# roryhighnam/iib_project_ldpc_codes

Measured on AMD Instinct MI355X. Metric: decoded codewords/sec + info-bit Gb/s, (3,6) n=10k 50-iter BP, 1/2/4/8 MI355X, higher is better.
Workload: dtype f32

## Files before the change

iib_project_ldpc_codes_amd/csrc/bp_loc.hpp:

```cpp
#pragma once
#include "bp_device.hpp"

namespace ldpc {
namespace {

#ifndef LDPC_LOC_VGROUP
#define LDPC_LOC_VGROUP 1
#endif
#ifndef LDPC_LOC_CGROUP
#define LDPC_LOC_CGROUP 1
#endif
template <int N, int D>
__device__ __forceinline__ uint32_t bits_parity(const float2 (&x)[D], bool hi, uint32_t seed) {
    auto w = [&](int j) { return __float_as_uint(hi ? x[j].y : x[j].x); };
    uint32_t p = seed;
    int j = 2;
#pragma unroll
    for (; j + 1 < N; j += 2) p = xor3u(p, w(j), w(j + 1));
    if (j < N) p ^= w(j);
    return p;
}
template <int D, int ALGO, bool MIXED = false, bool SGN = false, int CL = 0>
__device__ __forceinline__ int loc_check_pair(float *msg, int W, int Nc, int i, float2 &l0, float2 &l1, float alpha,
                                              uint32_t lpar = 0u, float2 *chain = nullptr) {
    constexpr int C = CL > 0 ? 1 : 0, U = D - 2 - C;
    float2 x[D];
    x[0] = l0;
    x[1] = l1;
    if constexpr (C) x[2] = *chain;
#pragma unroll
    for (int r = 0; r < U / 2; ++r) {
        const float4 f = *reinterpret_cast<const float4 *>(msg + W + r * 4 * Nc + 4 * i);
        x[2 + C + 2 * r] = make_float2(f.x, f.y);
        x[3 + C + 2 * r] = make_float2(f.z, f.w);
    }
    if constexpr (U % 2) x[D - 1] = *reinterpret_cast<const float2 *>(msg + W + (U / 2) * 4 * Nc + 2 * i);
    int unsat = 0;
    if constexpr (SGN) {
        unsat = (int)(bits_parity<MIXED ? D - 1 : D, D>(x, false, lpar) | bits_parity<D, D>(x, true, lpar >> 1));
    }
    if constexpr (ALGO == 0) {
        if constexpr (MIXED) {
            x[D - 1].x = 0.0f;
            check_update_spa_pair_rwire<D, true>(x);
        } else {
            check_update_spa_pair_rwire<D>(x);
        }
    } else {
        float xa[D], xb[D];
#pragma unroll
        for (int j = 0; j < D; ++j) { xa[j] = x[j].x; xb[j] = x[j].y; }
        if constexpr (MIXED) {
            xa[D - 1] = __builtin_inff();
            check_update<1, D>(xa, alpha);
            check_update<1, D>(xb, alpha);
        } else if constexpr (D == 6) {
            check_update_ms6(xa, alpha);
            check_update_ms6(xb, alpha);
        } else {
            check_update<1, D>(xa, alpha);
            check_update<1, D>(xb, alpha);
        }
#pragma unroll
        for (int j = 0; j < D; ++j) x[j] = make_float2(xa[j], xb[j]);
    }
#pragma unroll
    for (int r = 0; r < U / 2; ++r)
        *reinterpret_cast<float4 *>(msg + W + r * 4 * Nc + 4 * i) =
            make_float4(x[2 + C + 2 * r].x, x[2 + C + 2 * r].y, x[3 + C + 2 * r].x, x[3 + C + 2 * r].y);
    if constexpr (U % 2) *reinterpret_cast<float2 *>(msg + W + (U / 2) * 4 * Nc + 2 * i) = x[D - 1];
    l0 = x[0];
    l1 = x[1];
    if constexpr (C) *chain = x[2];
    return unsat;
}

template <int D, int DHI, int ALGO, bool SGN>
__device__ __forceinline__ int loc_check_dispatch(int code, float *msg, int W, int Nc, int i, float2 &l0, float2 &l1,
                                                  float alpha, uint32_t lpar) {
    if constexpr (D == DHI) {
        if (code >> 8) return loc_check_pair<D, ALGO, true, SGN>(msg, W, Nc, i, l0, l1, alpha, lpar);
        return loc_check_pair<D, ALGO, false, SGN>(msg, W, Nc, i, l0, l1, alpha, lpar);
    } else {
        if (code == D) return loc_check_pair<D, ALGO, false, SGN>(msg, W, Nc, i, l0, l1, alpha, lpar);
        return loc_check_dispatch<D + 1, DHI, ALGO, SGN>(code, msg, W, Nc, i, l0, l1, alpha, lpar);
    }
}

template <typename V>
__device__ __forceinline__ V ld_fresh(const V *p, int idx) {
    asm volatile("" : "+v"(idx));
    return p[idx];
}

__device__ __forceinline__ bool block_any(int pred, uint32_t *flag, int par) {
    if (__builtin_amdgcn_ballot_w64(pred != 0) != 0 && (threadIdx.x & (kWave - 1)) == 0) flag[par] = 1u;
    __syncthreads();
    const bool any = flag[par] != 0u;
    if (threadIdx.x == 0) flag[par ^ 1] = 0u;
    return any;
}
__device__ __forceinline__ uint32_t block_count(int pred, uint32_t *flag, int par) {
    const uint64_t bal = __builtin_amdgcn_ballot_w64(pred != 0);
    if (bal != 0 && (threadIdx.x & (kWave - 1)) == 0) atomicAdd(&flag[par], (uint32_t)__popcll(bal));
    __syncthreads();
    const uint32_t c = flag[par];
    if (threadIdx.x == 0) flag[par ^ 1] = 0u;
    return c;
}
#ifndef LDPC_LOC_EP_W0
#define LDPC_LOC_EP_W0 48
#endif
#ifndef LDPC_LOC_PRIO
#define LDPC_LOC_PRIO 1
#endif


constexpr int loc_waves_per_simd(int T, int KP) { return T == 512 && KP <= 5 ? 4 : 1; }

template <int DLO, int DHI, int DVN0, int DVN1, int KP, int T, int ALGO, bool ABS0, bool ABS1, bool ET = false,
          bool MC = false, bool EP = false, int CL = 0>
__global__ __launch_bounds__(T, loc_waves_per_simd(T, KP)) void bp_loc_kernel(BpArgs a) {
    static_assert(CL == 0 || (CL == KP - 1 && ALGO == 0 && !ET && !MC && !EP && DLO == DHI && DVN1 == 2 && !ABS1),
                  "chained layout: fixed-count sum-product on the one-class shape");
    auto chained = [](int v) { return CL > 0 && (v & 1) && (v >> 1) < CL; };
    float2 chain[CL > 0 ? CL : 1];
    static_assert(!ET || ALGO == 0 || DLO == DHI, "min-sum early stop: one check class");
    static_assert(!ET || 2 * 2 * KP <= 64, "early stop keeps the thread's decisions in one 64-bit word");
    constexpr bool MSET = ET && ALGO == 1;
    constexpr bool SGN_LSB = ET && ALGO == 0;
    constexpr int VP = 2 * KP;
    constexpr int DVM = DVN0 > DVN1 ? DVN0 : DVN1;
    constexpr int DVA = DVM > 0 ? DVM : 1;
    constexpr int DVP = DVA;
    extern __shared__ __align__(16) unsigned char smem[];
    __shared__ uint32_t stop_flag[2];
    float *msg = reinterpret_cast<float *>(smem);
    const int tid = threadIdx.x;
    const int n = a.n, iters = a.max_iters;
    const int lpos0 = (int)((uint32_t)(size_t)(lds_u8 *)smem >> 2);
    const uint32_t base2 = (uint32_t)lpos0 | ((uint32_t)lpos0 << 16);
    constexpr bool SPA = ALGO == 0;
    constexpr bool INF0 = ABS0 || ALGO == 1, INF1 = ABS1 || ALGO == 1;
    uint32_t sp[VP][DVA];
    uint32_t inf[VP];
    auto load_sp = [&](int v, int u) {
        return (uint32_t)ld_fresh(a.loc_pos, (v * DVP + u) * T + tid) + base2;
    };
    auto load_vars = [&](int (&vv)[2 * VP]) {
#pragma unroll
        for (int i = 0; i < 2 * VP; ++i) vv[i] = ld_fresh(a.loc_var, i * T + tid);
    };
#pragma unroll
    for (int k = 0; k < KP; ++k) {
        if constexpr (INF0) inf[2 * k] = (uint32_t)a.loc_info[(2 * k) * T + tid];
        if constexpr (INF1) inf[2 * k + 1] = (uint32_t)a.loc_info[(2 * k + 1) * T + tid];
    }
    auto at = [](uint32_t ba) -> lds_f32 & { return *(lds_f32 *)(size_t)ba; };
    const float neutral = SPA ? 1.0f : 0.0f;

    auto gather = [&](auto dn_tag, auto abs_tag, int v, const uint32_t (&spv)[DVA], float2 (&cv)[DVA],
                      uint32_t (&a0)[DVA], uint32_t (&a1)[DVA]) {
        constexpr int DN = decltype(dn_tag)::value;
        constexpr bool AB = decltype(abs_tag)::value;
        const int nl = chained(v) ? DN - 1 : DN;
#pragma unroll
        for (int u = 0; u < DN; ++u)
            if (u < nl) {
                a0[u] = pos_lo_x4(spv[u]);
                a1[u] = pos_hi_x4(spv[u]);
            }
#pragma unroll
        for (int u = 0; u < DN; ++u)
            if (u < nl) cv[u] = make_float2(at(a0[u]), at(a1[u]));
        if (chained(v)) cv[DN - 1] = chain[v >> 1];
        if constexpr (AB) {
#pragma unroll
            for (int u = 0; u < DN; ++u) {
                cv[u].x = (inf[v] >> u) & 1u ? cv[u].x : neutral;
                cv[u].y = (inf[v] >> (u + 4)) & 1u ? cv[u].y : neutral;
            }
        }
    };
    auto ms_sum = [&](auto dn_tag, int v, const float2 &Lv, const float2 &lv, const float2 (&cv)[DVA]) {
        constexpr int DN = decltype(dn_tag)::value;
        if constexpr (DN == 2) {
            float s2[2];
#pragma unroll
            for (int h = 0; h < 2; ++h) {
                const uint32_t e0 = (uint32_t)__builtin_amdgcn_sbfe((int)inf[v], 16 + 4 * h, 1);
                const uint32_t e2 = (uint32_t)__builtin_amdgcn_sbfe((int)inf[v], 18 + 4 * h, 1);
                const uint32_t ml = __float_as_uint(h ? lv.y : lv.x);
                const uint32_t n0 = __float_as_uint(h ? cv[0].y : cv[0].x), n1 = __float_as_uint(h ? cv[1].y : cv[1].x);
                const float a0 = __uint_as_float(bfi_u32(e0, ml, n0));
                const uint32_t u = bfi_u32(e0, n0, ml);
                const float a1 = __uint_as_float(bfi_u32(e2, n1, u));
                const float a2 = __uint_as_float(bfi_u32(e2, ml, n1));
                s2[h] = (((h ? Lv.y : Lv.x) + a0) + a1) + a2;
            }
            return make_float2(s2[0], s2[1]);
        }
        float s2[2];
#pragma unroll
        for (int h = 0; h < 2; ++h) {
            const int jl = (inf[v] >> (8 + 2 * h)) & 3;
            const float ml = h ? lv.y : lv.x;
            float s = h ? Lv.y : Lv.x;
#pragma unroll
            for (int j = 0; j <= DN; ++j) {
                const float nl = j == 0 ? 0.0f : (h ? cv[j - 1].y : cv[j - 1].x);
                const float nl2 = j < DN ? (h ? cv[j].y : cv[j].x) : 0.0f;
                s += j < jl ? nl2 : (j == jl ? ml : nl);
            }
            s2[h] = s;
        }
        return make_float2(s2[0], s2[1]);
    };

    int *curve = reinterpret_cast<int *>(smem + (((size_t)(a.loc_words + 64 > n ? a.loc_words + 64 : n) * 4 + 15) &
                                                  ~(size_t)15));
    uint32_t *syn = reinterpret_cast<uint32_t *>(reinterpret_cast<unsigned char *>(curve) +
                                                 (((size_t)(iters + 1) * 4 + 15) & ~(size_t)15));
    const int nsw = (2 * a.loc_P + 31) >> 5;
    using HB = std::conditional_t<(4 * KP > 32), uint64_t, uint32_t>;
    static_assert(!MSET || sizeof(HB) == 4, "MSET: 32-bit decision word");
    HB hbits = 0;
    HB lpar = 0;
    uint32_t chm = 0u;
    auto syn_flush = [&]() {
        uint32_t mk = chm;
        chm = 0u;
        const uint32_t P4 = 4u * (uint32_t)a.loc_P;
        constexpr int NF = 2;
        while (__builtin_amdgcn_ballot_w64(mk != 0u)) {
            int bit[NF];
            bool on[NF];
            uint32_t raw[NF][DVA];
#pragma unroll
            for (int f = 0; f < NF; ++f) {
                bit[f] = mk ? (int)__builtin_ctz(mk) : 0;
                on[f] = mk != 0u && tid + (bit[f] >> 2) * T < a.loc_P;
                mk &= mk - 1u;
            }
#pragma unroll
            for (int f = 0; f < NF; ++f)
#pragma unroll
                for (int u = 0; u < DVM; ++u) raw[f][u] = (uint32_t)a.loc_pos[((bit[f] >> 1) * DVP + u) * T + tid];
#pragma unroll
            for (int f = 0; f < NF; ++f) {
                if (on[f]) {
                    const int v = bit[f] >> 1, h = bit[f] & 1;
                    const int q = tid + (v >> 1) * T;
                    const uint32_t bl = 2u * (uint32_t)q + (uint32_t)h;
                    atomicXor(&syn[bl >> 5], 1u << (bl & 31));
                    const int dn = (v & 1) ? DVN1 : DVN0;
#pragma unroll
                    for (int u = 0; u < DVM; ++u) {
                        if (u < dn) {
                            uint32_t w = __builtin_amdgcn_ubfe(raw[f][u], 16u * (uint32_t)h, 16u);
                            w = w >= P4 ? w - P4 : w;
                            const uint32_t bn = 2u * (w >> 2) + (w & 1u);
                            atomicXor(&syn[bn >> 5], 1u << (bn & 31));
                        }
                    }
                }
            }
        }
    };
    static_assert(!EP || (ET && !MC), "EP: early-stop decodes with posteriors");
    constexpr bool ep = EP;
    float2 *slab = ep ? reinterpret_cast<float2 *>(a.scratch) + (size_t)blockIdx.x * VP * T : nullptr;
    __shared__ int next_b;
    const bool per = a.work != nullptr;
    uint32_t claim = 0u;
    for (int round = 0;; ++round) {
        if (per && tid == 0) next_b = round == 0 ? (int)atomicAdd(a.work, 1u) : (int)claim;
        __syncthreads();
        const int b = per ? __builtin_amdgcn_readfirstlane(next_b) : (int)blockIdx.x + round * (int)gridDim.x;
        if (b >= a.B) break;
        if (per && tid == 0) claim = atomicAdd(a.work, 1u);
        const uint64_t cw = a.first_cw + (uint64_t)b;
        int redo_it = -1;
    restart:
        int slab_it = -2;
        bool slab_now = false;
        if constexpr (ET) {
            if (tid == 0) stop_flag[0] = stop_flag[1] = 0u;
        }
        int err0 = 0;
        if constexpr (MC) {
            for (int i = tid; i <= iters; i += T) curve[i] = 0;
            if constexpr (MSET)
                for (int i = tid; i < nsw; i += T) syn[i] = 0u;
            for (int g4 = tid; g4 < (n + 3) >> 2; g4 += T) {
                const uint4 r = chan_block(a.ch, cw, g4);
#pragma unroll
                for (int q = 0; q < 4; ++q) {
                    if (4 * g4 + q >= n) break;
                    const float l = chan_soft_word(a.ch, r, q);
                    msg[4 * g4 + q] = to_msg<ALGO>(l);
                    err0 += (l < 0.0f);
                }
            }
        } else {
            if constexpr (MSET)
                for (int i = tid; i < nsw; i += T) syn[i] = 0u;
            for (int v = tid; v < n; v += T) msg[v] = to_msg<ALGO>(a.llr[(size_t)b * n + v]);
        }
        __syncthreads();
        if constexpr (MC) {
            const int w = wave_sum(err0);
            if ((tid & (kWave - 1)) == 0) atomicAdd(&curve[0], w);
        }
#pragma unroll
        for (int k = 0; k < KP; ++k) {
#pragma unroll
            for (int u = 0; u < DVN0; ++u) sp[2 * k][u] = load_sp(2 * k, u);
#pragma unroll
            for (int u = 0; u < DVN1; ++u)
                if (!(chained(2 * k + 1) && u == DVN1 - 1)) sp[2 * k + 1][u] = load_sp(2 * k + 1, u);
        }
        float2 L[VP];
        if constexpr (MC) {
            int vv[2 * VP];
            load_vars(vv);
#pragma unroll
            for (int v = 0; v < VP; ++v)
                L[v] = make_float2(vv[2 * v] >= 0 ? msg[vv[2 * v]] : 0.0f, vv[2 * v + 1] >= 0 ? msg[vv[2 * v + 1]] : 0.0f);
        } else {
#pragma unroll
            for (int v = 0; v < VP; ++v) {
                const int v0 = ld_fresh(a.loc_var, (v * 2 + 0) * T + tid), v1 = ld_fresh(a.loc_var, (v * 2 + 1) * T + tid);
                L[v] = make_float2(v0 >= 0 ? msg[v0] : 0.0f, v1 >= 0 ? msg[v1] : 0.0f);
            }
        }
        __syncthreads();
        float2 loc[VP];
        auto init = [&](auto dn_tag, int v) {
            constexpr int DN = decltype(dn_tag)::value;
            float2 w;
            if constexpr (SPA) {
                w = make_float2(__builtin_amdgcn_exp2f(__builtin_amdgcn_fmed3f(L[v].x, -23.0f, 23.0f)),
                                __builtin_amdgcn_exp2f(__builtin_amdgcn_fmed3f(L[v].y, -23.0f, 23.0f)));
                if constexpr (ET)
                    w = make_float2(__uint_as_float(bfi_lsb(__float_as_uint(w.x), (uint32_t)(L[v].x < 0.0f))),
                                    __uint_as_float(bfi_lsb(__float_as_uint(w.y), (uint32_t)(L[v].y < 0.0f))));
                L[v] = make_float2(__builtin_amdgcn_exp2f(__builtin_amdgcn_fmed3f(L[v].x, -126.0f, 126.0f)),
                                   __builtin_amdgcn_exp2f(__builtin_amdgcn_fmed3f(L[v].y, -126.0f, 126.0f)));
            } else {
                w = L[v];
                if constexpr (MSET) {
                    const int d0 = (int)(w.x < 0.0f) | ((int)(w.y < 0.0f) << 1);
                    hbits |= (uint32_t)d0 << (2 * v);
                    chm |= (uint32_t)d0 << (2 * v);
                }
            }
            loc[v] = w;
#pragma unroll
            for (int u = 0; u < DN; ++u) {
                if (chained(v) && u == DN - 1) {
                    chain[v >> 1] = w;
                } else {
                    at(pos_lo_x4(sp[v][u])) = w.x;
                    at(pos_hi_x4(sp[v][u])) = w.y;
                }
            }
        };
        hbits = 0u;
#pragma unroll
        for (int k = 0; k < KP; ++k) {
            init(int_c<DVN0>{}, 2 * k);
            init(int_c<DVN1>{}, 2 * k + 1);
        }
        if constexpr (MSET) syn_flush();
        auto var_pair = [&](auto dn_tag, auto abs_tag, int v) -> int {
            constexpr int DN = decltype(dn_tag)::value;
            constexpr int DV = DN + 1;
            uint32_t a0[DVA], a1[DVA];
            float2 cv[DVA];
            gather(dn_tag, abs_tag, v, sp[v], cv, a0, a1);
            int dec = 0;
            if constexpr (SPA) {
                float2 pre[DV];
                pre[0] = L[v];
                if constexpr (DV > 1) pre[1] = pre[0] * loc[v];
#pragma unroll
                for (int j = 2; j < DV; ++j) pre[j] = pre[j - 1] * cv[j - 2];
                uint32_t sx = 0, sy = 0;
                if constexpr (MC || ET) {
                    const float2 P = DN > 0 ? pre[DV - 1] * cv[DN > 0 ? DN - 1 : 0] : pre[DV - 1];
                    const uint32_t dx = (__float_as_uint(P.x) + 0xC0800000u) >> 31;
                    const uint32_t dy = (__float_as_uint(P.y) + 0xC0800000u) >> 31;
                    dec = (int)(dx | dy << 1);
                    if constexpr (ET) {
                        sx = dx;
                        sy = dy;
                    }
                }
                auto sgn = [&](float2 R) {
                    if constexpr (ET)
                        return make_float2(__uint_as_float(bfi_lsb(__float_as_uint(R.x), sx)),
                                           __uint_as_float(bfi_lsb(__float_as_uint(R.y), sy)));
                    return R;
                };
                float2 suf = DN > 0 ? cv[DN > 0 ? DN - 1 : 0] : make_float2(1.0f, 1.0f);
#pragma unroll
                for (int j = DV - 1; j >= 1; --j) {
                    const float2 R = sgn(ratio_wire2(j == DV - 1 ? pre[j] : pre[j] * suf));
                    if (chained(v) && j == DV - 1) {
                        chain[v >> 1] = R;
                    } else {
                        at(a0[j - 1]) = R.x;
                        at(a1[j - 1]) = R.y;
                    }
                    if (j < DV - 1) suf = suf * cv[j - 1];
                }
                if (ep && slab_now) slab[v * T + tid] = loc[v] * suf;
                loc[v] = ratio_wire2(DN > 0 ? L[v] * suf : L[v]);
            } else {
                const float2 s = ms_sum(dn_tag, v, L[v], loc[v], cv);
                if (ep && slab_now) slab[v * T + tid] = s;
#pragma unroll
                for (int u = 0; u < DN; ++u) {
                    at(a0[u]) = s.x - cv[u].x;
                    at(a1[u]) = s.y - cv[u].y;
                }
                loc[v] = make_float2(s.x - loc[v].x, s.y - loc[v].y);
                if constexpr (MC || ET)
                    dec = (int)((__float_as_uint(s.x) >> 31) | ((__float_as_uint(s.y) >> 31) << 1));
            }
            return dec;
        };
        int it = 0;
        bool stopped = false;
        for (; it < iters; ++it) {
            __syncthreads();
            int unsat = 0;
            {
#pragma unroll
                for (int v = 0; v < VP; ++v)
#pragma unroll
                    for (int u = 0; u < DVA; ++u)
                        if (!(chained(v) && u == DVA - 1)) asm volatile("" : "+v"(sp[v][u]));
            }
            if constexpr (ALGO == 1) {
#pragma unroll
                for (int v = 0; v < VP; ++v) asm volatile("" : "+v"(inf[v]));
            }
            if (LDPC_LOC_PRIO) __builtin_amdgcn_s_setprio(0);
            if constexpr (CL > 0) {
                const int Tq = a.loc_cls_q[1];
                if (tid < Tq) {
#pragma unroll
                    for (int k = 0; k < KP; ++k) {
                        int i = tid + (k > 0 ? (k - 1) * Tq : 0);
                        asm volatile("" : "+v"(i));
                        if (k == 0)
                            loc_check_pair<DLO, ALGO>(msg, 0, Tq, i, loc[0], loc[1], a.alpha);
                        else
                            loc_check_pair<DLO, ALGO, false, false, CL>(msg, a.loc_cls_w[1], (KP - 1) * Tq, i, loc[2 * k],
                                                                        loc[2 * k + 1], a.alpha, 0u, &chain[k - 1]);
                        if (LDPC_LOC_CGROUP > 0 && k % LDPC_LOC_CGROUP == LDPC_LOC_CGROUP - 1)
                            __builtin_amdgcn_sched_barrier(0);
                    }
                }
            }
#pragma unroll
            for (int k = 0; k < (CL > 0 ? 0 : KP); ++k) {
                int q = tid + k * T;
                asm volatile("" : "+v"(q));
                if (q < a.loc_P) {
                    if constexpr (DLO == DHI) {
                        unsat |= loc_check_pair<DLO, ALGO, false, ET && SPA>(msg, 0, a.loc_P, q, loc[2 * k],
                                                                             loc[2 * k + 1], a.alpha,
                                                                             (uint32_t)(lpar >> (4 * k)));
                    } else {
                        int q0 = a.loc_cls_q[0], q1 = a.loc_cls_q[1], W = a.loc_cls_w[0], d = a.loc_cls_d[0];
#pragma unroll
                        for (int j = 1; j < 4; ++j) {
                            const bool in = j < a.loc_ncls && q >= a.loc_cls_q[j];
                            q0 = in ? a.loc_cls_q[j] : q0;
                            q1 = in ? a.loc_cls_q[j + 1] : q1;
                            W = in ? a.loc_cls_w[j] : W;
                            d = in ? a.loc_cls_d[j] : d;
                        }
                        unsat |= loc_check_dispatch<DLO, DHI, ALGO, ET && SPA>(d, msg, W, q1 - q0, q - q0, loc[2 * k],
                                                                               loc[2 * k + 1], a.alpha,
                                                                               (uint32_t)(lpar >> (4 * k)));
                    }
                }
                if (LDPC_LOC_CGROUP > 0 && k % LDPC_LOC_CGROUP == LDPC_LOC_CGROUP - 1)
                    __builtin_amdgcn_sched_barrier(0);
            }
            if constexpr (MSET)
                for (int i = tid; i < nsw; i += T) unsat |= syn[i] != 0u;
            if constexpr (ET) {
                if constexpr (SGN_LSB) unsat &= 1;
                bool more;
                if constexpr (EP) {
                    const uint32_t cnt = block_count(unsat | (it == 0), stop_flag, it & 1);
                    more = cnt != 0u;
                    slab_now = cnt <= (uint32_t)LDPC_LOC_EP_W0 || it == redo_it;
                    if (more && slab_now) slab_it = it;
                } else {
                    more = block_any(unsat | (it == 0), stop_flag, it & 1);
                }
                if (!more) {
                    stopped = true;
                    break;
                }
            } else {
                __syncthreads();
            }
            if (!MC && it == iters - 1) break;
            if (LDPC_LOC_PRIO) __builtin_amdgcn_s_setprio(1);
            int errs = 0;
            HB nh = 0;
            {
#pragma unroll
                for (int k = 0; k < KP; ++k) {
                    const int d0 = var_pair(int_c<DVN0>{}, bool_c<ABS0>{}, 2 * k);
                    if (LDPC_LOC_VGROUP == 1) __builtin_amdgcn_sched_barrier(0);
                    const int d1 = var_pair(int_c<DVN1>{}, bool_c<ABS1>{}, 2 * k + 1);
                    if (LDPC_LOC_VGROUP > 0) __builtin_amdgcn_sched_barrier(0);
                    if constexpr (ET) nh |= (HB)(d0 | d1 << 2) << (4 * k);
                    else if constexpr (MC) errs += tid + k * T < a.loc_P ? __builtin_popcount(d0) + __builtin_popcount(d1) : 0;
                }
            }
            if constexpr (ET) {
                if constexpr (MSET) chm = (uint32_t)(nh ^ hbits);
                hbits = nh;
                if constexpr (SGN_LSB) lpar = nh ^ (nh >> 2);
                if constexpr (MC) {
                    const int lim = a.loc_P - tid, nk = lim <= 0 ? 0 : min(KP, (lim + T - 1) / T);
                    const HB vm = 4 * nk >= 8 * (int)sizeof(HB) ? ~(HB)0 : (((HB)1 << (4 * nk)) - 1);
                    errs = sizeof(HB) == 8 ? __builtin_popcountll((uint64_t)(nh & vm)) : __builtin_popcount((uint32_t)(nh & vm));
                }
                if constexpr (MSET) syn_flush();
            }
            if constexpr (MC) {
                const int w = wave_sum(errs);
                if ((tid & (kWave - 1)) == 0) atomicAdd(&curve[it + 1], w);
            }
        }
        if constexpr (MC) {
            __syncthreads();
            int32_t *tr = a.trial + (size_t)b * (iters + 1);
            const int last = curve[it];
            for (int i = tid; i <= iters; i += T) tr[i] = i <= it ? curve[i] : last;
            if (tid == 0) a.its[b] = it;
            continue;
        }
        if constexpr (ET && !MC) {
            if (stopped && ep && slab_it != it - 1) {
                redo_it = it - 1;
                __syncthreads();
                goto restart;
            }
            if (stopped && ep) {
                uint8_t *hb = reinterpret_cast<uint8_t *>(msg + n);
#pragma unroll
                for (int v = 0; v < VP; ++v) {
                    const float2 q = slab[v * T + tid];
                    float2 pv;
                    if constexpr (SPA) {
                        pv = make_float2(__builtin_amdgcn_logf(L[v].x) + __builtin_amdgcn_logf(q.x),
                                         __builtin_amdgcn_logf(L[v].y) + __builtin_amdgcn_logf(q.y));
                    } else {
                        pv = q;
                    }
                    const int v0 = ld_fresh(a.loc_var, (v * 2 + 0) * T + tid), v1 = ld_fresh(a.loc_var, (v * 2 + 1) * T + tid);
                    if constexpr (SPA) {
                        const float lx = __builtin_amdgcn_logf(L[v].x), ly = __builtin_amdgcn_logf(L[v].y);
                        if (v0 >= 0 && fabsf(lx) >= 125.5f) pv.x = to_msg<ALGO>(a.llr[(size_t)b * n + v0]) + __builtin_amdgcn_logf(q.x);
                        if (v1 >= 0 && fabsf(ly) >= 125.5f) pv.y = to_msg<ALGO>(a.llr[(size_t)b * n + v1]) + __builtin_amdgcn_logf(q.y);
                    }
                    if (v0 >= 0) {
                        msg[v0] = pv.x;
                        hb[v0] = (uint8_t)((hbits >> (2 * v)) & 1);
                    }
                    if (v1 >= 0) {
                        msg[v1] = pv.y;
                        hb[v1] = (uint8_t)((hbits >> (2 * v + 1)) & 1);
                    }
                }
                __syncthreads();
                for (int v = tid; v < n; v += T) {
                    a.post[(size_t)b * n + v] = msg[v] * Domain<ALGO>::out;
                    if (a.hard) a.hard[(size_t)b * n + v] = hb[v];
                }
                if (a.its && tid == 0) a.its[b] = it;
                continue;
            }
        }
        if constexpr (ET) {
            if (stopped) {
#pragma unroll
                for (int v = 0; v < VP; ++v) {
                    const int v0 = ld_fresh(a.loc_var, (v * 2 + 0) * T + tid), v1 = ld_fresh(a.loc_var, (v * 2 + 1) * T + tid);
                    if (v0 >= 0) msg[v0] = (hbits >> (2 * v)) & 1 ? -1.0f : 1.0f;
                    if (v1 >= 0) msg[v1] = (hbits >> (2 * v + 1)) & 1 ? -1.0f : 1.0f;
                }
                __syncthreads();
                if (a.hard)
                    for (int v = tid; v < n; v += T) a.hard[(size_t)b * n + v] = (uint8_t)(msg[v] < 0.0f);
                if (a.its && tid == 0) a.its[b] = it;
                continue;
            }
        }
        float2 pr[VP];
        auto post = [&](auto dn_tag, auto abs_tag, int v) {
            constexpr int DN = decltype(dn_tag)::value;
            uint32_t a0[DVA], a1[DVA], spv[DVA];
            float2 cv[DVA];
#pragma unroll
            for (int u = 0; u < DN; ++u)
                if (!(chained(v) && u == DN - 1)) spv[u] = load_sp(v, u);
            gather(dn_tag, abs_tag, v, spv, cv, a0, a1);
            if constexpr (SPA) {
                float2 s;
                s = make_float2(__builtin_amdgcn_logf(L[v].x), __builtin_amdgcn_logf(L[v].y));
                if (fabsf(s.x) >= 125.5f || fabsf(s.y) >= 125.5f) {
                    const float *lb = a.llr + (size_t)b * n;
                    const int v0 = ld_fresh(a.loc_var, (v * 2 + 0) * T + tid);
                    const int v1 = ld_fresh(a.loc_var, (v * 2 + 1) * T + tid);
                    if (fabsf(s.x) >= 125.5f && v0 >= 0) s.x = to_msg<ALGO>(lb[v0]);
                    if (fabsf(s.y) >= 125.5f && v1 >= 0) s.y = to_msg<ALGO>(lb[v1]);
                }
                s = s + make_float2(__builtin_amdgcn_logf(loc[v].x), __builtin_amdgcn_logf(loc[v].y));
#pragma unroll
                for (int u = 0; u < DN; ++u)
                    s = s + make_float2(__builtin_amdgcn_logf(cv[u].x), __builtin_amdgcn_logf(cv[u].y));
                pr[v] = s;
            } else {
                pr[v] = ms_sum(dn_tag, v, L[v], loc[v], cv);
            }
            __builtin_amdgcn_sched_barrier(0);
        };
#pragma unroll
        for (int k = 0; k < KP; ++k) {
            post(int_c<DVN0>{}, bool_c<ABS0>{}, 2 * k);
            post(int_c<DVN1>{}, bool_c<ABS1>{}, 2 * k + 1);
        }
        __syncthreads();
#pragma unroll
        for (int v = 0; v < VP; ++v) {
            const int v0 = ld_fresh(a.loc_var, (v * 2 + 0) * T + tid), v1 = ld_fresh(a.loc_var, (v * 2 + 1) * T + tid);
            if (v0 >= 0) msg[v0] = pr[v].x;
            if (v1 >= 0) msg[v1] = pr[v].y;
        }
        __syncthreads();
        for (int v = tid; v < n; v += T) {
            const float s = msg[v];
            if (a.post) a.post[(size_t)b * n + v] = s * Domain<ALGO>::out;
            if (a.hard) a.hard[(size_t)b * n + v] = (uint8_t)(s < 0.0f);
        }
        if (a.its && tid == 0) a.its[b] = iters;
    }
}

template <int DLO, int DHI, int D0, int D1, bool A0, bool A1, int T, int KP, int ALGO, bool ET, bool MC>
hipError_t launch_loc_shape(const BpPlan &p, BpArgs a, hipStream_t s) {
    auto launch = [&](auto k) {
        hipError_t e = allow_lds(k, p.lds);
        if (e != hipSuccess) return e;
        if (p.persistent) {
            a.work = reinterpret_cast<uint32_t *>(reinterpret_cast<char *>(a.scratch) + p.counter);
            if ((e = hipMemsetAsync(a.work, 0, sizeof(uint32_t), s)) != hipSuccess) return e;
        }
        hipLaunchKernelGGL(k, dim3(p.grid), dim3(T), p.lds, s, a);
        return hipGetLastError();
    };
    if constexpr (ET && !MC) {
        if (a.post) return launch(bp_loc_kernel<DLO, DHI, D0, D1, KP, T, ALGO, A0, A1, true, false, true>);
    }
    return launch(bp_loc_kernel<DLO, DHI, D0, D1, KP, T, ALGO, A0, A1, ET, MC>);
}

template <int DLO, int DHI, int D0, int D1, bool A0, bool A1, int ALGO, bool ET, bool MC>
hipError_t launch_loc_deg(const BpPlan &p, const BpArgs &a, int T, int KP, hipStream_t s) {
#define LOC_SHAPE(TT, KK) \
    if (T == TT && KP == KK) return launch_loc_shape<DLO, DHI, D0, D1, A0, A1, TT, KK, ALGO, ET, MC>(p, a, s);
    LOC_SHAPE(256, 1) LOC_SHAPE(256, 2) LOC_SHAPE(256, 3) LOC_SHAPE(256, 4)
    LOC_SHAPE(1024, 2) LOC_SHAPE(1024, 3)
    if constexpr (DLO != DHI) {
        LOC_SHAPE(512, 8) LOC_SHAPE(512, 10)
    } else {
        LOC_SHAPE(512, 5)
    }
#undef LOC_SHAPE
    return hipErrorInvalidValue;
}

template <int ALGO, bool ET, bool MC>
hipError_t launch_loc_modes(const BpPlan &p, const ldpc_graph &g, BpArgs a, hipStream_t s) {
    if (p.chain) {
        if constexpr (ALGO == 0 && !ET && !MC) {
            constexpr int KP = kLocChainKP, T = kLocChainT;
            if (g.chn_Tq <= 0 || g.chn_Tq > T || g.loc_P != KP * g.chn_Tq || !g.chn_var || !g.chn_pos)
                return hipErrorInvalidValue;
            a.loc_var = g.chn_var;
            a.loc_pos = g.chn_pos;
            a.loc_info = g.chn_info;
            a.loc_P = g.loc_P;
            a.loc_ncls = 2;
            a.loc_words = g.chn_words;
            a.loc_cls_q[0] = 0; a.loc_cls_q[1] = g.chn_Tq; a.loc_cls_q[2] = g.loc_P;
            a.loc_cls_w[0] = 0; a.loc_cls_w[1] = 8 * g.chn_Tq; a.loc_cls_w[2] = g.chn_words;
            a.loc_cls_d[0] = a.loc_cls_d[1] = 6;
            auto k = bp_loc_kernel<6, 6, 2, 2, KP, T, 0, false, false, false, false, false, kLocChainCL>;
            const hipError_t e = allow_lds(k, p.lds);
            if (e != hipSuccess) return e;
            hipLaunchKernelGGL(k, dim3(p.grid), dim3(T), p.lds, s, a);
            return hipGetLastError();
        } else {
            return hipErrorInvalidValue;
        }
    }
    a.loc_var = g.loc_var;
    a.loc_pos = g.loc_pos;
    a.loc_info = g.loc_info;
    a.loc_P = g.loc_P;
    a.loc_ncls = g.loc_ncls;
    a.loc_words = g.loc_words;
    for (int i = 0; i < 5; ++i) {
        a.loc_cls_q[i] = g.loc_cls_q[i];
        a.loc_cls_w[i] = g.loc_cls_w[i];
    }
    for (int i = 0; i < 4; ++i) a.loc_cls_d[i] = g.loc_cls_d[i];
    const int variant = loc_variant(g.loc_dlo, g.loc_dhi, g.loc_DVN, g.loc_dvn0, g.loc_dvn1, g.loc_abs0, g.loc_abs1,
                                    g.loc_T, g.loc_KP);
    if (variant == kLocReg36) return launch_loc_deg<6, 6, 2, 2, false, false, ALGO, ET, MC>(p, a, g.loc_T, g.loc_KP, s);
    if (variant == kLocNone) return hipErrorInvalidValue;
    if constexpr (ET && ALGO == 1) return hipErrorInvalidValue;
    else return launch_loc_deg<5, 6, 1, 3, false, true, ALGO, ET, MC>(p, a, g.loc_T, g.loc_KP, s);
}

template <int ALGO>
hipError_t launch_loc_algo(const BpPlan &p, const ldpc_graph &g, const BpArgs &a, bool et, bool mc, hipStream_t s) {
    if (mc) return et ? launch_loc_modes<ALGO, true, true>(p, g, a, s) : launch_loc_modes<ALGO, false, true>(p, g, a, s);
    return et ? launch_loc_modes<ALGO, true, false>(p, g, a, s) : launch_loc_modes<ALGO, false, false>(p, g, a, s);
}

}
}
```

Before: 2.539 million.

## Stage LLR loads, hoist index tables, and register-cache var ids in local BP kernel

When chained layout is enabled, the sparse-table and variable-index loads are issued before the LLR staging. The LLR load is unrolled into a fixed-count register batch so global latency overlaps. In the fixed-iteration path, the posterior stage reuses the preloaded sp tables and keeps variable ids in registers instead of reloading them from global memory. The SPA clamp-substitution branch is hoisted into a wave-uniform ballot so the common path carries no per-variable fallback code. The final output write loop is unrolled the same way, at the cost of extra register pressure that may reduce occupancy.

```diff
diff --git a/iib_project_ldpc_codes_amd/csrc/bp_loc.hpp b/iib_project_ldpc_codes_amd/csrc/bp_loc.hpp
--- a/iib_project_ldpc_codes_amd/csrc/bp_loc.hpp
+++ b/iib_project_ldpc_codes_amd/csrc/bp_loc.hpp
@@ -287,6 +287,22 @@
         if constexpr (ET) {
             if (tid == 0) stop_flag[0] = stop_flag[1] = 0u;
         }
+        constexpr bool STG = CL > 0;
+        auto load_tabs = [&]() {
+#pragma unroll
+            for (int k = 0; k < KP; ++k) {
+#pragma unroll
+                for (int u = 0; u < DVN0; ++u) sp[2 * k][u] = load_sp(2 * k, u);
+#pragma unroll
+                for (int u = 0; u < DVN1; ++u)
+                    if (!(chained(2 * k + 1) && u == DVN1 - 1)) sp[2 * k + 1][u] = load_sp(2 * k + 1, u);
+            }
+        };
+        int vv[2 * VP];
+        if constexpr (STG) {
+            load_tabs();
+            load_vars(vv);
+        }
         int err0 = 0;
         if constexpr (MC) {
             for (int i = tid; i <= iters; i += T) curve[i] = 0;
@@ -305,25 +321,29 @@
         } else {
             if constexpr (MSET)
                 for (int i = tid; i < nsw; i += T) syn[i] = 0u;
-            for (int v = tid; v < n; v += T) msg[v] = to_msg<ALGO>(a.llr[(size_t)b * n + v]);
+            if constexpr (STG) {
+                float r[2 * VP];
+                const float *lb = a.llr + (size_t)b * n;
+                int t = tid;
+                asm volatile("" : "+v"(t));
+#pragma unroll
+                for (int i = 0; i < 2 * VP; ++i) r[i] = lb[min(t + i * T, n - 1)];
+#pragma unroll
+                for (int i = 0; i < 2 * VP; ++i)
+                    if (t + i * T < n) msg[t + i * T] = to_msg<ALGO>(r[i]);
+            } else {
+                for (int v = tid; v < n; v += T) msg[v] = to_msg<ALGO>(a.llr[(size_t)b * n + v]);
+            }
         }
         __syncthreads();
         if constexpr (MC) {
             const int w = wave_sum(err0);
             if ((tid & (kWave - 1)) == 0) atomicAdd(&curve[0], w);
         }
-#pragma unroll
-        for (int k = 0; k < KP; ++k) {
-#pragma unroll
-            for (int u = 0; u < DVN0; ++u) sp[2 * k][u] = load_sp(2 * k, u);
-#pragma unroll
-            for (int u = 0; u < DVN1; ++u)
-                if (!(chained(2 * k + 1) && u == DVN1 - 1)) sp[2 * k + 1][u] = load_sp(2 * k + 1, u);
-        }
+        if constexpr (!STG) load_tabs();
         float2 L[VP];
-        if constexpr (MC) {
-            int vv[2 * VP];
-            load_vars(vv);
+        if constexpr (MC || STG) {
+            if constexpr (!STG) load_vars(vv);
 #pragma unroll
             for (int v = 0; v < VP; ++v)
                 L[v] = make_float2(vv[2 * v] >= 0 ? msg[vv[2 * v]] : 0.0f, vv[2 * v + 1] >= 0 ? msg[vv[2 * v + 1]] : 0.0f);
@@ -339,7 +359,12 @@
         auto init = [&](auto dn_tag, int v) {
             constexpr int DN = decltype(dn_tag)::value;
             float2 w;
-            if constexpr (SPA) {
+            if constexpr (SPA && STG) {
+                L[v] = make_float2(__builtin_amdgcn_exp2f(__builtin_amdgcn_fmed3f(L[v].x, -126.0f, 126.0f)),
+                                   __builtin_amdgcn_exp2f(__builtin_amdgcn_fmed3f(L[v].y, -126.0f, 126.0f)));
+                w = make_float2(__builtin_amdgcn_fmed3f(L[v].x, 0x1p-23f, 0x1p23f),
+                                __builtin_amdgcn_fmed3f(L[v].y, 0x1p-23f, 0x1p23f));
+            } else if constexpr (SPA) {
                 w = make_float2(__builtin_amdgcn_exp2f(__builtin_amdgcn_fmed3f(L[v].x, -23.0f, 23.0f)),
                                 __builtin_amdgcn_exp2f(__builtin_amdgcn_fmed3f(L[v].y, -23.0f, 23.0f)));
                 if constexpr (ET)
@@ -608,19 +633,41 @@
                 continue;
             }
         }
+        constexpr bool FIX = !ET && !MC;
         float2 pr[VP];
-        auto post = [&](auto dn_tag, auto abs_tag, int v) {
+        int pid[2 * VP];
+        bool clamped = false;
+        if constexpr (FIX) {
+            load_vars(pid);
+            if constexpr (SPA) {
+#pragma unroll
+                for (int v = 0; v < VP; ++v)
+                    clamped |= fabsf(__builtin_amdgcn_logf(L[v].x)) >= 125.5f || fabsf(__builtin_amdgcn_logf(L[v].y)) >= 125.5f;
+            }
+        }
+        auto post = [&](auto dn_tag, auto abs_tag, auto subst_tag, int v) {
             constexpr int DN = decltype(dn_tag)::value;
+            constexpr bool SUBST = decltype(subst_tag)::value;
             uint32_t a0[DVA], a1[DVA], spv[DVA];
             float2 cv[DVA];
-#pragma unroll
-            for (int u = 0; u < DN; ++u)
-                if (!(chained(v) && u == DN - 1)) spv[u] = load_sp(v, u);
-            gather(dn_tag, abs_tag, v, spv, cv, a0, a1);
+            if constexpr (FIX) {
+                gather(dn_tag, abs_tag, v, sp[v], cv, a0, a1);
+            } else {
+#pragma unroll
+                for (int u = 0; u < DN; ++u)
+                    if (!(chained(v) && u == DN - 1)) spv[u] = load_sp(v, u);
+                gather(dn_tag, abs_tag, v, spv, cv, a0, a1);
+            }
             if constexpr (SPA) {
                 float2 s;
                 s = make_float2(__builtin_amdgcn_logf(L[v].x), __builtin_amdgcn_logf(L[v].y));
-                if (fabsf(s.x) >= 125.5f || fabsf(s.y) >= 125.5f) {
+                if constexpr (FIX) {
+                    if constexpr (SUBST) {
+                        const float *lb = a.llr + (size_t)b * n;
+                        if (fabsf(s.x) >= 125.5f && pid[2 * v] >= 0) s.x = to_msg<ALGO>(lb[pid[2 * v]]);
+                        if (fabsf(s.y) >= 125.5f && pid[2 * v + 1] >= 0) s.y = to_msg<ALGO>(lb[pid[2 * v + 1]]);
+                    }
+                } else if (fabsf(s.x) >= 125.5f || fabsf(s.y) >= 125.5f) {
                     const float *lb = a.llr + (size_t)b * n;
                     const int v0 = ld_fresh(a.loc_var, (v * 2 + 0) * T + tid);
                     const int v1 = ld_fresh(a.loc_var, (v * 2 + 1) * T + tid);
@@ -637,23 +684,54 @@
             }
             __builtin_amdgcn_sched_barrier(0);
         };
-#pragma unroll
-        for (int k = 0; k < KP; ++k) {
-            post(int_c<DVN0>{}, bool_c<ABS0>{}, 2 * k);
-            post(int_c<DVN1>{}, bool_c<ABS1>{}, 2 * k + 1);
+        if (FIX && SPA && __builtin_expect(__builtin_amdgcn_ballot_w64(clamped) != 0, 0)) {
+#pragma unroll
+            for (int k = 0; k < KP; ++k) {
+                post(int_c<DVN0>{}, bool_c<ABS0>{}, bool_c<true>{}, 2 * k);
+                post(int_c<DVN1>{}, bool_c<ABS1>{}, bool_c<true>{}, 2 * k + 1);
+            }
+        } else {
+#pragma unroll
+            for (int k = 0; k < KP; ++k) {
+                post(int_c<DVN0>{}, bool_c<ABS0>{}, bool_c<false>{}, 2 * k);
+                post(int_c<DVN1>{}, bool_c<ABS1>{}, bool_c<false>{}, 2 * k + 1);
+            }
         }
         __syncthreads();
 #pragma unroll
         for (int v = 0; v < VP; ++v) {
-            const int v0 = ld_fresh(a.loc_var, (v * 2 + 0) * T + tid), v1 = ld_fresh(a.loc_var, (v * 2 + 1) * T + tid);
+            int v0, v1;
+            if constexpr (FIX) {
+                v0 = pid[2 * v];
+                v1 = pid[2 * v + 1];
+            } else {
+                v0 = ld_fresh(a.loc_var, (v * 2 + 0) * T + tid);
+                v1 = ld_fresh(a.loc_var, (v * 2 + 1) * T + tid);
+            }
             if (v0 >= 0) msg[v0] = pr[v].x;
             if (v1 >= 0) msg[v1] = pr[v].y;
         }
         __syncthreads();
-        for (int v = tid; v < n; v += T) {
-            const float s = msg[v];
-            if (a.post) a.post[(size_t)b * n + v] = s * Domain<ALGO>::out;
-            if (a.hard) a.hard[(size_t)b * n + v] = (uint8_t)(s < 0.0f);
+        if constexpr (FIX) {
+            float o[2 * VP];
+            int t = tid;
+            asm volatile("" : "+v"(t));
+#pragma unroll
+            for (int i = 0; i < 2 * VP; ++i) o[i] = msg[min(t + i * T, n - 1)];
+#pragma unroll
+            for (int i = 0; i < 2 * VP; ++i) {
+                const int v = t + i * T;
+                if (v < n) {
+                    if (a.post) a.post[(size_t)b * n + v] = o[i] * Domain<ALGO>::out;
+                    if (a.hard) a.hard[(size_t)b * n + v] = (uint8_t)(o[i] < 0.0f);
+                }
+            }
+        } else {
+            for (int v = tid; v < n; v += T) {
+                const float s = msg[v];
+                if (a.post) a.post[(size_t)b * n + v] = s * Domain<ALGO>::out;
+                if (a.hard) a.hard[(size_t)b * n + v] = (uint8_t)(s < 0.0f);
+            }
         }
         if (a.its && tid == 0) a.its[b] = iters;
     }
```

New measurement: 2.567 million, median of 6. 1.01x the previous value.
